# ml-unito/PartitionedLS.jl

Measured on NVIDIA B200. Metric: opt_fit_orthant_nnls_solves_per_sec, higher is better.
Workload: dtype f64

## Files before the change

partitionedls.jl_b200/csrc/nnls5.cu:

```cuda
#include "common.cuh"

namespace pls {
namespace {

constexpr int H5_BYTES_ = 192;
constexpr int SG_FREE5 = 2;
constexpr unsigned char ST_INO = 1;
constexpr unsigned char ST_PAS = 2;
constexpr unsigned char ST_BLK = 4;
constexpr unsigned char ST_FAST = 8;
#define SYNC5() __syncthreads()

__device__ __forceinline__ void dmma5(double &d0, double &d1, double a, double b) {
  asm("mma.sync.aligned.m8n8k4.row.col.f64.f64.f64.f64 {%0,%1}, {%2}, {%3}, {%0,%1};\n"
      : "+d"(d0), "+d"(d1) : "d"(a), "d"(b));
}
__device__ __forceinline__ double rcp5(double x) {
  double r;
  asm("rcp.approx.ftz.f64 %0, %1;" : "=d"(r) : "d"(x));
  double e = fma(-x, r, 1.0);
  r = fma(r, e, r);
  e = fma(-x, r, 1.0);
  return fma(r, e, r);
}
__device__ __forceinline__ double wsum5(double v) {
#pragma unroll
  for (int o = 16; o; o >>= 1) v += __shfl_xor_sync(0xffffffffu, v, o);
  return v;
}
__device__ __forceinline__ double wmax5(double v) {
#pragma unroll
  for (int o = 16; o; o >>= 1) v = fmax(v, __shfl_xor_sync(0xffffffffu, v, o));
  return v;
}
__host__ __device__ constexpr int t2_doubles(int nr) { return ((nr / 8) * (nr / 8 + 1) / 2) * 64; }
__device__ __forceinline__ int t2_idx(int i, int j) {
  const int ti = i >> 3, tj = j >> 3;
  return ((((ti * (ti + 1)) >> 1) + tj) << 6) + ((i & 7) << 3) + (j & 7);
}
__device__ __forceinline__ double t2_get(const double *T2, int i, int j) { return i >= j ? T2[t2_idx(i, j)] : T2[t2_idx(j, i)]; }
__device__ __forceinline__ void t2_set(double *T2, int i, int j, double v) {
  const int a = i > j ? i : j, b = i > j ? j : i;
  const int x = t2_idx(a, b);
  T2[x] = v;
  if ((a >> 3) == (b >> 3)) T2[x - ((a & 7) << 3) - (b & 7) + ((b & 7) << 3) + (a & 7)] = v;
}
__device__ __forceinline__ int pan5(int row, int col) { return (row << 3) + (col ^ ((row & 2) << 1)); }

struct Sh5 {
  double *T2;
  double *v;
  double *Pp, *Wp;
  double *yv;
  double *D;
  double *gd;
  double *red;
  int4 *binfo;
  int *ctl;
  short *slot;
  short *rvar;
  short *lst;
  short *lstE;
  short *lstB;
  unsigned short *tmap;
  signed char *sg;
  unsigned char *st;
  unsigned char *grp;
  unsigned char *mk;
};
enum { C_NS = 0, C_OK, C_CNT, C_N, C_NJ, C_NP, C_NLV, C_FLAG };

__host__ __device__ inline size_t sh5_bytes(int NR, int ld1) {
  const int ntl = (NR / 8) * (NR / 8 + 1) / 2;
  return H5_BYTES_ + sizeof(double) * ((size_t)t2_doubles(NR) + ld1 + 16 * (size_t)NR + NR + 64 + 8 + 32 + 16) + sizeof(int) * 16 +
         sizeof(short) * (2 * (size_t)ld1 + 2 * (size_t)NR + 8 + ((ntl + 3) & ~3)) + 3 * (size_t)ld1 + NR + 16 + 16;
}

__device__ __forceinline__ Sh5 make_sh5(int NR, int ld1) {
  extern __shared__ __align__(16) unsigned char smem_raw5[];
  const int ntl = (NR / 8) * (NR / 8 + 1) / 2;
  Sh5 s;
  double *dp = reinterpret_cast<double *>(smem_raw5 + H5_BYTES_);
  s.T2 = dp; dp += t2_doubles(NR);
  s.Pp = dp; dp += 8 * NR;
  s.Wp = dp; dp += 8 * NR;
  s.yv = dp; dp += NR;
  s.D = dp; dp += 64;
  s.gd = dp; dp += 8;
  s.red = dp; dp += 32;
  s.binfo = reinterpret_cast<int4 *>(dp); dp += 16;
  int *ip = reinterpret_cast<int *>(dp);
  s.ctl = ip; ip += 16;
  short *sp = reinterpret_cast<short *>(ip);
  s.rvar = sp; sp += NR;
  s.lstE = sp; sp += NR;
  s.lstB = sp; sp += 8;
  s.tmap = reinterpret_cast<unsigned short *>(sp); sp += (ntl + 3) & ~3;
  s.mk = reinterpret_cast<unsigned char *>(sp);
  dp = reinterpret_cast<double *>(smem_raw5 + ((static_cast<int>(s.mk - smem_raw5) + NR + 15) & ~15));
  s.v = dp; dp += ld1;
  sp = reinterpret_cast<short *>(dp);
  s.slot = sp; sp += ld1;
  s.lst = sp; sp += ld1;
  signed char *cp = reinterpret_cast<signed char *>(sp);
  s.sg = cp; cp += ld1;
  s.st = reinterpret_cast<unsigned char *>(cp); cp += ld1;
  s.grp = reinterpret_cast<unsigned char *>(cp);
  return s;
}

struct H5 {
  double *T1;
  const double *T1r;
  double *Pg;
  const double *G;
  const unsigned long long *gmask;
  int ld1, nr, Mp, ldg;
  int cold_fused;
  int gen;
  int pad0, pad1;
  unsigned long long cnt[10];
  double yy, cmax;
  double max_viol;
};
enum { H_SWEEP = 0, H_STREAM, H_SUMS, H_SUMP2, H_ITER, H_BLK, H_REBUILD, H_FOLD, H_DRIFT, H_NOCONV };
constexpr int H5_BYTES = H5_BYTES_;
static_assert(sizeof(H5) <= H5_BYTES, "header size");
__device__ __forceinline__ H5 &hdr5() {
  extern __shared__ __align__(16) unsigned char smem_raw5[];
  return *reinterpret_cast<H5 *>(smem_raw5);
}

template <int T>
__device__ __forceinline__ double bmax5(const Sh5 &s, double v) {
  constexpr int NW = T / 32;
  v = wmax5(v);
  if ((threadIdx.x & 31) == 0) s.red[threadIdx.x >> 5] = v;
  SYNC5();
  double r = s.red[0];
#pragma unroll
  for (int i = 1; i < NW; ++i) r = fmax(r, s.red[i]);
  SYNC5();
  return r;
}

template <int T>
__device__ __forceinline__ void set_block5(const Sh5 &s, int nb, int slot) {
  const int tid = threadIdx.x;
  const H5 &h = hdr5();
  const int g = h.gen;
  if (g == 1) {
    #pragma unroll 1
    for (int k = tid; k < h.nr; k += T) s.mk[k] = 0;
    SYNC5();
  }
  if (tid < nb) {
    const int tc = slot >> 3, c7 = slot & 7;
    s.lstB[tid] = (short)slot;
    s.binfo[tid] = make_int4(slot, (tc << 6) + c7, (((tc * (tc + 1)) >> 1) << 6) + (c7 << 3), 0);
    s.mk[slot] = (unsigned char)g;
  }
}

template <int T, int NR>
__device__ __noinline__ int t2_block(int n, int nb, int nlv, bool test, bool flip) {
  H5 &h = hdr5();
  const int gen = h.gen;
  const Sh5 s = make_sh5(NR, h.ld1);
  constexpr int NW = T / 32;
  const int tid = threadIdx.x, lane = tid & 31, wid = tid >> 5;
  const int fr = lane >> 2, fk = lane & 3;
  const int ntr = (n + 7) >> 3;
  const short *B = s.lstB;
  if (tid >= 32 || T == 32) {
    constexpr int TG = T == 32 ? 32 : T - 32;
#pragma unroll 1
    for (int row = T == 32 ? tid : tid - 32; row < ntr * 8; row += TG) {
      const int tr = row >> 3, r7 = row & 7;
      const int rbase = (((tr * (tr + 1)) >> 1) << 6) + (r7 << 3), rowt = (tr << 6) + r7;
      const int sw = (row & 2) << 1, pb = row << 3;
#pragma unroll 1
      for (int q = 0; q < 8; ++q) {
        double val = 0.0;
        if (row < n && q < nb) { const int4 bi = s.binfo[q]; val = s.T2[row >= bi.x ? rbase + bi.y : bi.z + rowt]; }
        s.Pp[pb + (q ^ sw)] = val;
      }
    }
  }
  if (tid < 32) {
    if (lane < 8) {
      s.gd[lane] = (test && lane >= nlv && lane < nb) ? 1e-13 * __ldg(h.G + (size_t)h.ldg * s.rvar[B[lane]] + s.rvar[B[lane]]) : 0.0;
    }
    const int i = lane >> 2, j0 = (lane & 3) << 1;
    double e0 = (i < nb && j0 < nb) ? t2_get(s.T2, B[i], B[j0]) : (i == j0 ? 1.0 : 0.0);
    double e1 = (i < nb && j0 + 1 < nb) ? t2_get(s.T2, B[i], B[j0 + 1]) : (i == j0 + 1 ? 1.0 : 0.0);
    int bad = nb;
#pragma unroll 1
    for (int k = 0; k < nb; ++k) {
      __syncwarp();
      s.D[i * 8 + j0] = e0; s.D[i * 8 + j0 + 1] = e1;
      __syncwarp();
      const double pk0 = s.D[k * 8 + j0], pk1 = s.D[k * 8 + j0 + 1], cik = s.D[i * 8 + k], pkk = s.D[k * 8 + k];
      const bool good = k < nlv ? pkk < 0.0 : (test ? pkk > s.gd[k] : pkk > 0.0);
      if (!good && bad == nb) bad = k;
      const double d = rcp5(pkk), fct = cik * d;
      const bool rowk = i == k;
      double n0 = rowk ? pk0 * d : fma(-fct, pk0, e0);
      double n1 = rowk ? pk1 * d : fma(-fct, pk1, e1);
      if (j0 == k) n0 = rowk ? d : -fct;
      if (j0 + 1 == k) n1 = rowk ? d : -fct;
      e0 = n0; e1 = n1;
    }
    __syncwarp();
    s.D[i * 8 + j0] = e0; s.D[i * 8 + j0 + 1] = e1;
    if (lane == 0) s.ctl[C_OK] = bad == nb ? nb : (bad < nlv ? -1 : bad);
  }
  SYNC5();
  const int res = s.ctl[C_OK];
  if (tid == 0) h.gen = gen == 255 ? 1 : gen + 1;
  if (res != nb) { SYNC5(); return res; }
  #pragma unroll 1
  for (int ti = wid; ti < ntr; ti += NW) {
    double c0 = 0.0, c1 = 0.0;
    dmma5(c0, c1, s.Pp[pan5(ti * 8 + fr, fk)], s.D[fk * 8 + fr]);
    dmma5(c0, c1, s.Pp[pan5(ti * 8 + fr, 4 + fk)], s.D[(4 + fk) * 8 + fr]);
    *reinterpret_cast<double2 *>(s.Wp + pan5(ti * 8 + fr, 2 * fk)) = make_double2(c0, c1);
  }
  SYNC5();
  {
    const int ntl = (ntr * (ntr + 1)) >> 1;
    int q = (ntl * wid) / NW;
    const int q1 = (ntl * (wid + 1)) / NW;
    const int t0 = s.tmap[q];
    int ti = t0 >> 8, tj = t0 & 255;
    const int la0 = pan5(fr, fk), la1 = pan5(fr, 4 + fk);
    double2 *cp = reinterpret_cast<double2 *>(s.T2 + (q << 6) + fr * 8 + 2 * fk);
    const double *pw = s.Wp + (ti << 6), *pp = s.Pp + (tj << 6);
    double a0 = -pw[la0], a1 = -pw[la1];
#pragma unroll 1
    for (; q < q1; ++q) {
      double2 c0 = *cp;
      dmma5(c0.x, c0.y, a0, pp[la0]);
      dmma5(c0.x, c0.y, a1, pp[la1]);
      *cp = c0;
      cp += 32; pp += 64;
      if (++tj > ti) { ++ti; tj = 0; pp = s.Pp; pw += 64; a0 = -pw[la0]; a1 = -pw[la1]; }
    }
  }
  SYNC5();
#pragma unroll 1
  for (int row = tid; row < n; row += T) {
    if (s.mk[row] == (unsigned char)gen) continue;
    const int tr = row >> 3, r7 = row & 7;
    const int rbase = (((tr * (tr + 1)) >> 1) << 6) + (r7 << 3), rowt = (tr << 6) + r7;
    const int sw = (row & 2) << 1, pb = row << 3;
#pragma unroll 1
    for (int q = 0; q < nb; ++q) {
      const int4 bi = s.binfo[q];
      const int tc = bi.x >> 3;
      const double w0 = s.Wp[pb + (q ^ sw)];
      const double val = q < nlv ? -w0 : w0;
      if (tr >= tc) s.T2[rbase + bi.y] = val;
      if (tr <= tc) s.T2[bi.z + rowt] = val;
    }
  }
#pragma unroll 1
  for (int e = tid; e < 64; e += T) {
    const int i = e >> 3, j = e & 7;
    if (i < nb && j <= i) { const double val = s.D[i * 8 + j]; t2_set(s.T2, B[i], B[j], ((i < nlv) == (j < nlv)) ? -val : val); }
  }
  if (flip && tid < nb) s.st[s.rvar[B[tid]]] ^= ST_PAS;
  SYNC5();
  if (tid == 0) { h.cnt[H_SWEEP] += nb; h.cnt[H_SUMP2] += ((unsigned long long)(n * n) * nb) >> 2; }
  return nb;
}

template <int T, int NR>
__device__ __noinline__ bool t2_rebuild(int n) {
  const H5 &h = hdr5();
  const Sh5 s = make_sh5(NR, h.ld1);
  constexpr int NW = T / 32;
  const int tid = threadIdx.x, lane = tid & 31, wid = tid >> 5;
  #pragma unroll 1
  for (int i = wid; i < n; i += NW) {
    const double *row = h.T1r + (size_t)h.ld1 * s.rvar[i];
    #pragma unroll 1
    for (int j = lane; j <= i; j += 32) t2_set(s.T2, i, j, __ldcg(row + s.rvar[j]));
  }
  if (tid < 32) {
    int cnt = 0, nlv = 0;
    #pragma unroll 1
    for (int pass = 0; pass < 2; ++pass) {
      #pragma unroll 1
      for (int k0 = 1; k0 < n; k0 += 32) {
        const int k = k0 + lane;
        bool take = false;
        if (k < n) { const unsigned char f = s.st[s.rvar[k]]; const bool pas = f & ST_PAS, ino = f & ST_INO; take = pas != ino && (pass == 0 ? !pas : pas); }
        const unsigned bal = __ballot_sync(0xffffffffu, take);
        if (take) s.lst[cnt + __popc(bal & ((1u << lane) - 1))] = (short)k;
        cnt += __popc(bal);
      }
      if (pass == 0) nlv = cnt;
    }
    if (lane == 0) { s.ctl[C_CNT] = cnt; s.ctl[C_NLV] = nlv; }
  }
  SYNC5();
  const int cnt = s.ctl[C_CNT], nlv = s.ctl[C_NLV];
  #pragma unroll 1
  for (int q0 = 0; q0 < cnt; q0 += 8) {
    const int nb = min(8, cnt - q0);
    set_block5<T>(s, nb, tid < nb ? s.lst[q0 + tid] : 0);
    SYNC5();
    if (t2_block<T, NR>(n, nb, max(0, min(nb, nlv - q0)), false, false) != nb) return false;
  }
  return true;
}

template <int NR>
__device__ __noinline__ int window_reset() {
  const H5 &h = hdr5();
  const Sh5 s = make_sh5(NR, h.ld1);
  const int tid = threadIdx.x;
  const int Mp = h.Mp;
  if (tid < 32) {
    const int lane = tid;
    if (lane == 0) s.rvar[0] = (short)Mp;
    int base = 1;
    #pragma unroll 1
    for (int m0 = 0; m0 < Mp; m0 += 32) {
      const int m = m0 + lane;
      bool keep = false;
      if (m < Mp) {
        const unsigned char f = s.st[m];
        keep = (f & ST_FAST) || (((f & ST_PAS) != 0) != ((f & ST_INO) != 0));
      }
      const unsigned bal = __ballot_sync(0xffffffffu, keep);
      if (m < Mp) {
        if (keep) { const int k = base + __popc(bal & ((1u << lane) - 1)); s.rvar[k] = (short)m; s.slot[m] = (short)k; }
        else s.slot[m] = -1;
      }
      base += __popc(bal);
    }
    if (lane == 0) s.ctl[C_N] = base;
  }
  SYNC5();
  return s.ctl[C_N];
}

template <int T, int NR>
__device__ __noinline__ int t2_compact(int n) {
  const H5 &h = hdr5();
  const Sh5 s = make_sh5(NR, h.ld1);
  const int tid = threadIdx.x;
  double *scr = h.Pg + 8 * (size_t)h.ld1;
  short *old = s.lst;
  if (tid < 32) {
    const int lane = tid;
    if (lane == 0) old[0] = 0;
    int base = 1;
    #pragma unroll 1
    for (int k0 = 1; k0 < n; k0 += 32) {
      const int k = k0 + lane;
      bool keep = false; int m = 0;
      if (k < n) {
        m = s.rvar[k];
        const unsigned char f = s.st[m];
        keep = (f & ST_FAST) || (((f & ST_PAS) != 0) != ((f & ST_INO) != 0));
      }
      const unsigned bal = __ballot_sync(0xffffffffu, keep);
      const int kn = base + __popc(bal & ((1u << lane) - 1));
      __syncwarp();
      if (k < n) {
        if (keep) { old[kn] = (short)k; s.rvar[kn] = (short)m; s.slot[m] = (short)kn; }
        else s.slot[m] = -1;
      }
      __syncwarp();
      base += __popc(bal);
    }
    if (lane == 0) s.ctl[C_N] = base;
  }
  SYNC5();
  const int nn = s.ctl[C_N];
  if (nn == n) return n;
  #pragma unroll 1
  for (int idx = tid; idx < nn * nn; idx += T) {
    const int a = idx / nn, b = idx - a * nn;
    if (b <= a) __stcg(scr + idx, t2_get(s.T2, old[a], old[b]));
  }
  __threadfence_block();
  SYNC5();
  #pragma unroll 1
  for (int idx = tid; idx < nn * nn; idx += T) {
    const int a = idx / nn, b = idx - a * nn;
    if (b <= a) t2_set(s.T2, a, b, __ldcg(scr + idx));
  }
  SYNC5();
  return nn;
}

template <int T, int NQ, int NR>
__device__ __noinline__ void stream5(int n) {
  const H5 &h = hdr5();
  const Sh5 s = make_sh5(NR, h.ld1);
  const int tid = threadIdx.x;
  const int ld2 = h.ld1 >> 1;
  constexpr int UB = 8;
  constexpr int NG = T >= 512 ? 2 : 1, TG = T / NG, NQE = NQ * NG, UBG = UB * NG;
  const int grp = NG == 1 ? 0 : tid / TG, lt = NG == 1 ? tid : tid - grp * TG;
  int ns = 0;
  {
    constexpr int NW = T / 32;
    const int lane = tid & 31, wid = tid >> 5;
    int *ri = reinterpret_cast<int *>(s.red);
    #pragma unroll 1
    for (int k0 = 1; k0 < n; k0 += T) {
      const int k = k0 + tid;
      bool tg = false, pas = false; int m = 0;
      if (k < n) { m = s.rvar[k]; const unsigned char f = s.st[m]; pas = f & ST_PAS; tg = pas != ((f & ST_INO) != 0); }
      const unsigned bal = __ballot_sync(0xffffffffu, tg);
      if (k0 > 1) SYNC5();
      if (lane == 0) ri[wid] = __popc(bal);
      SYNC5();
      int off = ns;
#pragma unroll
      for (int w2 = 0; w2 < NW; ++w2) { const int c = ri[w2]; if (w2 < wid) off += c; ns += c; }
      if (tg) { const int p = off + __popc(bal & ((1u << lane) - 1)); s.lst[p] = (short)m; const double t = s.T2[t2_idx(k, 0)]; s.yv[p] = pas ? t : -t; }
    }
    const int nsp = (ns + UBG - 1) / UBG * UBG;
    #pragma unroll 1
    for (int p = ns + tid; p < nsp; p += T) { s.lst[p] = (short)h.Mp; s.yv[p] = 0.0; }
    if (tid == 0) { s.ctl[C_NS] = ns; s.ctl[C_FLAG] = 0; }
  }
  SYNC5();
  const int nsp = (ns + UBG - 1) / UBG * UBG;
  double2 acc[NQE];
  const double2 *T1v = reinterpret_cast<const double2 *>(h.T1r);
  {
    const double2 *r = T1v + (size_t)ld2 * h.Mp;
#pragma unroll
    for (int q = 0; q < NQE; ++q) acc[q] = (grp == 0 && lt + TG * q < ld2) ? __ldcg(r + lt + TG * q) : make_double2(0.0, 0.0);
  }
  #pragma unroll 1
  for (int p = 0; p < nsp; p += UBG) {
    double2 g[UB][NQE];
#pragma unroll
    for (int u = 0; u < UB; ++u) {
      const double2 *r = T1v + (size_t)ld2 * s.lst[p + u * NG + grp];
#pragma unroll
      for (int q = 0; q < NQE; ++q) g[u][q] = (lt + TG * q < ld2) ? __ldcg(r + lt + TG * q) : make_double2(0.0, 0.0);
    }
#pragma unroll
    for (int u = 0; u < UB; ++u) {
      const double y = s.yv[p + u * NG + grp];
#pragma unroll
      for (int q = 0; q < NQE; ++q) { acc[q].x = fma(-y, g[u][q].x, acc[q].x); acc[q].y = fma(-y, g[u][q].y, acc[q].y); }
    }
  }
  if (NG > 1) {
    double2 *scr = reinterpret_cast<double2 *>(s.Wp);
    if (grp == 1) {
#pragma unroll
      for (int q = 0; q < NQE; ++q) if (lt + TG * q < ld2) scr[lt + TG * q] = acc[q];
    }
    SYNC5();
    if (grp == 0) {
#pragma unroll
      for (int q = 0; q < NQE; ++q) if (lt + TG * q < ld2) { const double2 o = scr[lt + TG * q]; acc[q].x += o.x; acc[q].y += o.y; }
    }
  }
  if (grp == 0) {
#pragma unroll
    for (int q = 0; q < NQE; ++q)
      if (lt + TG * q < ld2) reinterpret_cast<double2 *>(s.v)[lt + TG * q] = acc[q];
  }
  SYNC5();
  if (tid == 0) { hdr5().cnt[H_STREAM]++; hdr5().cnt[H_SUMS] += ns; }
}

template <int T, int NR>
__device__ __noinline__ void join5(int n, int m) {
  const H5 &h = hdr5();
  const Sh5 s = make_sh5(NR, h.ld1);
  const int tid = threadIdx.x;
  const double *row1 = h.T1r + (size_t)h.ld1 * m;
  double *rowv = s.Wp, *tog = s.Wp + NR;
  int ns = 0;
  {
    constexpr int NW = T / 32;
    const int lane = tid & 31, wid = tid >> 5;
    int *ri = reinterpret_cast<int *>(s.red);
    #pragma unroll 1
    for (int k0 = 1; k0 < n; k0 += T) {
      const int k = k0 + tid;
      bool tg = false, pas = false; int var = 0;
      if (k < n) { var = s.rvar[k]; const unsigned char f = s.st[var]; pas = f & ST_PAS; tg = pas != ((f & ST_INO) != 0); }
      const unsigned bal = __ballot_sync(0xffffffffu, tg);
      if (k0 > 1) SYNC5();
      if (lane == 0) ri[wid] = __popc(bal);
      SYNC5();
      int off = ns;
#pragma unroll
      for (int w2 = 0; w2 < NW; ++w2) { const int c = ri[w2]; if (w2 < wid) off += c; ns += c; }
      if (tg) { const int p = off + __popc(bal & ((1u << lane) - 1)); s.lstE[p] = (short)k; const double a = __ldcg(row1 + var); s.yv[p] = pas ? a : -a; }
      if (k < n) tog[k] = tg ? 1.0 : 0.0;
    }
    if (tid == 0) tog[0] = 0.0;
  }
  SYNC5();
  #pragma unroll 1
  for (int j = tid; j < n; j += T) {
    double a = tog[j] != 0.0 ? 0.0 : __ldcg(row1 + s.rvar[j]);
    #pragma unroll 1
    for (int p = 0; p < ns; ++p) a = fma(-s.yv[p], t2_get(s.T2, s.lstE[p], j), a);
    rowv[j] = a;
  }
  SYNC5();
  #pragma unroll 1
  for (int j = tid; j < n; j += T) t2_set(s.T2, n, j, rowv[j]);
  if (tid < 32) {
    double dg = 0.0;
    #pragma unroll 1
    for (int p = tid; p < ns; p += 32) dg = fma(s.yv[p], rowv[s.lstE[p]], dg);
    dg = wsum5(dg);
    if (tid == 0) { t2_set(s.T2, n, n, __ldcg(row1 + m) - dg); s.rvar[n] = (short)m; s.slot[m] = (short)n; }
  }
  if (tid == 0) hdr5().cnt[H_SUMP2] += (unsigned long long)(ns * n) >> 1;
  SYNC5();
}

template <int T, int NR>
__device__ __noinline__ bool fold_block5(int boff, int nb) {
  H5 &h = hdr5();
  const Sh5 s = make_sh5(NR, h.ld1);
  const short *B = s.lstE + boff;
  constexpr int NW = T / 32;
  const int tid = threadIdx.x, lane = tid & 31, wid = tid >> 5;
  const int fr = lane >> 2, fk = lane & 3;
  const int ld1 = h.ld1, nt = ld1 >> 3;
  double *FP = s.T2, *FW = s.T2 + (size_t)ld1 * 8;
  #pragma unroll 1
  for (int idx = tid; idx < ld1 * 8; idx += T) {
    const int j = idx >> 3, q = idx & 7;
    FP[pan5(j, q)] = q < nb ? __ldcg(h.T1r + (size_t)ld1 * B[q] + j) : 0.0;
  }
  if (tid < 8) s.gd[tid] = (tid < nb && (s.st[B[tid]] & ST_PAS)) ? 1e-13 * __ldg(h.G + (size_t)h.ldg * B[tid] + B[tid]) : 0.0;
  SYNC5();
  if (tid < 32) {
    bool ok = true;
    const int i = lane >> 2, j0 = (lane & 3) << 1;
    double e0 = (i < nb && j0 < nb) ? FP[pan5(B[i], j0)] : (i == j0 ? 1.0 : 0.0);
    double e1 = (i < nb && j0 + 1 < nb) ? FP[pan5(B[i], j0 + 1)] : (i == j0 + 1 ? 1.0 : 0.0);
    #pragma unroll 1
    for (int k = 0; k < nb; ++k) {
      __syncwarp();
      s.D[i * 8 + j0] = e0; s.D[i * 8 + j0 + 1] = e1;
      __syncwarp();
      const double pk0 = s.D[k * 8 + j0], pk1 = s.D[k * 8 + j0 + 1], cik = s.D[i * 8 + k], pkk = s.D[k * 8 + k];
      if (s.st[B[k]] & ST_PAS) ok = ok && pkk > s.gd[k];
      else ok = ok && pkk < 0.0;
      const double d = 1.0 / pkk, fct = cik * d;
      const bool rowk = i == k;
      double n0 = rowk ? pk0 * d : fma(-fct, pk0, e0);
      double n1 = rowk ? pk1 * d : fma(-fct, pk1, e1);
      if (j0 == k) n0 = rowk ? d : -fct;
      if (j0 + 1 == k) n1 = rowk ? d : -fct;
      e0 = n0; e1 = n1;
    }
    __syncwarp();
    s.D[i * 8 + j0] = e0; s.D[i * 8 + j0 + 1] = e1;
    ok = __all_sync(0xffffffffu, ok);
    if (lane == 0) s.ctl[C_OK] = ok ? 1 : 0;
  }
  SYNC5();
  if (!s.ctl[C_OK]) { SYNC5(); return false; }
  #pragma unroll 1
  for (int ti = wid; ti < nt; ti += NW) {
    double c0 = 0.0, c1 = 0.0;
    dmma5(c0, c1, FP[pan5(ti * 8 + fr, fk)], s.D[fk * 8 + fr]);
    dmma5(c0, c1, FP[pan5(ti * 8 + fr, 4 + fk)], s.D[(4 + fk) * 8 + fr]);
    *reinterpret_cast<double2 *>(FW + pan5(ti * 8 + fr, 2 * fk)) = make_double2(c0, c1);
  }
  SYNC5();
  {
    const int ntl = (nt * (nt + 1)) >> 1;
    constexpr int IFL = (T <= 64 || T >= 512) ? 8 : 4;
    int q = (ntl * wid) / NW;
    const int q1 = (ntl * (wid + 1)) / NW;
    int ti = 0;
    while (((ti + 1) * (ti + 2)) >> 1 <= q) ++ti;
    int tj = q - ((ti * (ti + 1)) >> 1);
    #pragma unroll 1
    for (; q < q1; q += IFL) {
      double2 c[IFL]; int ri[IFL], rj[IFL];
#pragma unroll
      for (int u = 0; u < IFL; ++u) {
        ri[u] = ti; rj[u] = tj;
        c[u] = __ldcg(reinterpret_cast<const double2 *>(h.T1r + (size_t)(ti * 8 + fr) * ld1 + tj * 8 + 2 * fk));
        if (q + u + 1 < q1) { if (++tj > ti) { ++ti; tj = 0; } }
      }
#pragma unroll
      for (int u = 0; u < IFL; ++u) {
        const int ra = ri[u] * 8 + fr, rb = rj[u] * 8 + fr;
        dmma5(c[u].x, c[u].y, -FW[pan5(ra, fk)], FP[pan5(rb, fk)]);
        dmma5(c[u].x, c[u].y, -FW[pan5(ra, 4 + fk)], FP[pan5(rb, 4 + fk)]);
      }
#pragma unroll
      for (int u = 0; u < IFL; ++u) {
        if (q + u < q1) {
          __stcg(reinterpret_cast<double2 *>(h.T1 + (size_t)(ri[u] * 8 + fr) * ld1 + rj[u] * 8 + 2 * fk), c[u]);
          if (ri[u] != rj[u]) {
            double *mp = h.T1 + (size_t)(rj[u] * 8 + 2 * fk) * ld1 + ri[u] * 8 + fr;
            __stcg(mp, c[u].x); __stcg(mp + ld1, c[u].y);
          }
        }
      }
    }
  }
  SYNC5();
  #pragma unroll 1
  for (int idx = tid; idx < ld1 * 8; idx += T) {
    const int i = idx >> 3, q = idx & 7;
    if (q < nb) {
      const double val = (s.st[B[q]] & ST_PAS) ? FW[pan5(i, q)] : -FW[pan5(i, q)];
      __stcg(h.T1 + (size_t)ld1 * B[q] + i, val);
      __stcg(h.T1 + (size_t)ld1 * i + B[q], val);
    }
  }
  SYNC5();
  #pragma unroll 1
  for (int e = tid; e < 64; e += T) {
    const int i = e >> 3, j = e & 7;
    if (i < nb && j < nb) {
      const double ei = (s.st[B[i]] & ST_PAS) ? 1.0 : -1.0, ej = (s.st[B[j]] & ST_PAS) ? 1.0 : -1.0;
      __stcg(h.T1 + (size_t)ld1 * B[i] + B[j], -ei * ej * s.D[i * 8 + j]);
    }
  }
  SYNC5();
  if (tid < nb) { const int m = B[tid]; const unsigned char f = s.st[m]; s.st[m] = (f & ST_PAS) ? (unsigned char)(f | ST_INO) : (unsigned char)(f & ~ST_INO); }
  if (tid == 0) { h.T1r = h.T1; h.cnt[H_SUMP2] += 2ull * ld1 * ld1; h.cnt[H_FOLD]++; }
  SYNC5();
  return true;
}

template <int T, int NR>
__device__ __noinline__ void fold_fused5(int n) {
  H5 &h = hdr5();
  const Sh5 s = make_sh5(NR, h.ld1);
  constexpr int NW = T / 32;
  const int tid = threadIdx.x, lane = tid & 31, wid = tid >> 5;
  const int fr = lane >> 2, fk = lane & 3;
  const int ld1 = h.ld1, nt = ld1 >> 3;
  const int ntr = (n + 7) >> 3, nk = ntr << 3;
  double *PR = h.Pg + 8 * (size_t)ld1, *ZT = PR + (size_t)ld1 * h.nr;
  int *roff = reinterpret_cast<int *>(s.Wp);
  const bool own = h.T1r == h.T1;
  const double *rows = own ? PR : h.T1r;
  #pragma unroll 1
  for (int k = tid; k < nk; k += T) {
    double e = 0.0;
    if (k >= 1 && k < n) { const unsigned char f = s.st[s.rvar[k]]; const bool pas = f & ST_PAS, ino = f & ST_INO; if (pas != ino) e = pas ? 1.0 : -1.0; }
    s.yv[k] = e;
    roff[k] = e != 0.0 ? (own ? k : (int)s.rvar[k]) * ld1 : 0;
  }
  SYNC5();
  if (own) {
    #pragma unroll 1
    for (int k = 0; k < n; ++k) {
      if (k > 0 && s.yv[k] == 0.0) continue;
      const double *src = h.T1 + (size_t)ld1 * (s.yv[k] != 0.0 ? s.rvar[k] : 0);
      #pragma unroll 1
      for (int j = tid; j < ld1; j += T) PR[(size_t)k * ld1 + j] = __ldcg(src + j);
    }
    __threadfence_block();
    SYNC5();
  }
  constexpr int NTQ = 12;
#pragma unroll 1
  for (int tj = wid; tj < nt; tj += NW) {
    const double *pa = rows + tj * 8 + fr;
    double2 acc[NTQ];
#pragma unroll
    for (int u = 0; u < NTQ; ++u) acc[u] = make_double2(0.0, 0.0);
    double a0 = s.yv[fk] * __ldcg(pa + roff[fk]), a1 = s.yv[4 + fk] * __ldcg(pa + roff[4 + fk]);
#pragma unroll 1
    for (int tk = 0; tk < ntr; ++tk) {
      double n0 = 0.0, n1 = 0.0;
      if (tk + 1 < ntr) { const int k = (tk + 1) * 8 + fk; n0 = s.yv[k] * __ldcg(pa + roff[k]); n1 = s.yv[k + 4] * __ldcg(pa + roff[k + 4]); }
#pragma unroll
      for (int tq = 0; tq < NTQ; ++tq) {
        if (tq < ntr) {
          double b0, b1;
          if (tk >= tq) { const double *tp = s.T2 + ((((tk * (tk + 1)) >> 1) + tq) << 6); b0 = tp[fk * 8 + fr]; b1 = tp[(4 + fk) * 8 + fr]; }
          else { const double *tp = s.T2 + ((((tq * (tq + 1)) >> 1) + tk) << 6); b0 = tp[fr * 8 + fk]; b1 = tp[fr * 8 + 4 + fk]; }
          dmma5(acc[tq].x, acc[tq].y, a0, b0); dmma5(acc[tq].x, acc[tq].y, a1, b1);
        }
      }
      a0 = n0; a1 = n1;
    }
#pragma unroll
    for (int tq = 0; tq < NTQ; ++tq)
      if (tq < ntr) {
        const int k = tq * 8 + 2 * fk;
        *reinterpret_cast<double2 *>(ZT + (size_t)(tj * 8 + fr) * nk + k) = make_double2(acc[tq].x * s.yv[k], acc[tq].y * s.yv[k + 1]);
      }
  }
  __threadfence_block();
  SYNC5();
  constexpr int CH = 5;
  {
    const int ntl = (nt * (nt + 1)) >> 1;
    int q = (ntl * wid) / NW;
    const int q1 = (ntl * (wid + 1)) / NW;
    int ti = 0;
    while (((ti + 1) * (ti + 2)) >> 1 <= q) ++ti;
    int tj = q - ((ti * (ti + 1)) >> 1);
    #pragma unroll 1
    for (; q < q1; ++q) {
      double2 c = __ldcg(reinterpret_cast<const double2 *>(h.T1r + (size_t)(ti * 8 + fr) * ld1 + tj * 8 + 2 * fk));
      const double *za = ZT + (size_t)(ti * 8 + fr) * nk + fk, *pb = rows + tj * 8 + fr;
#pragma unroll 1
      for (int t0 = 0; t0 < ntr; t0 += CH) {
        double z0[CH], z1[CH], p0[CH], p1[CH];
#pragma unroll
        for (int u = 0; u < CH; ++u) {
          const bool live = t0 + u < ntr;
          const int k = (t0 + u) * 8 + fk;
          z0[u] = live ? za[(t0 + u) * 8] : 0.0; z1[u] = live ? za[(t0 + u) * 8 + 4] : 0.0;
          p0[u] = live ? __ldcg(pb + roff[k]) : 0.0; p1[u] = live ? __ldcg(pb + roff[k + 4]) : 0.0;
        }
#pragma unroll
        for (int u = 0; u < CH; ++u) { dmma5(c.x, c.y, z0[u], p0[u]); dmma5(c.x, c.y, z1[u], p1[u]); }
      }
      __stcg(reinterpret_cast<double2 *>(h.T1 + (size_t)(ti * 8 + fr) * ld1 + tj * 8 + 2 * fk), c);
      if (ti != tj) {
        double *mp = h.T1 + (size_t)(tj * 8 + 2 * fk) * ld1 + ti * 8 + fr;
        __stcg(mp, c.x); __stcg(mp + ld1, c.y);
      }
      if (++tj > ti) { ++ti; tj = 0; }
    }
  }
  SYNC5();
  #pragma unroll 1
  for (int k = 1; k < n; ++k) {
    const double e = s.yv[k];
    if (e == 0.0) continue;
    const int var = s.rvar[k];
    #pragma unroll 1
    for (int j = tid; j < ld1; j += T) {
      const double val = -e * ZT[(size_t)j * nk + k];
      __stcg(h.T1 + (size_t)ld1 * var + j, val);
      __stcg(h.T1 + (size_t)ld1 * j + var, val);
    }
  }
  SYNC5();
  #pragma unroll 1
  for (int idx = tid; idx < n * n; idx += T) {
    const int a = idx / n, b = idx - a * n;
    __stcg(h.T1 + (size_t)ld1 * s.rvar[a] + s.rvar[b], t2_get(s.T2, a, b));
  }
  SYNC5();
  #pragma unroll 1
  for (int k = tid; k < n; k += T) {
    if (k >= 1 && s.yv[k] != 0.0) { const int m = s.rvar[k]; const unsigned char f = s.st[m]; s.st[m] = (f & ST_PAS) ? (unsigned char)(f | ST_INO) : (unsigned char)(f & ~ST_INO); }
  }
  if (tid == 0) { h.T1r = h.T1; h.cnt[H_SUMP2] += 2ull * ld1 * ld1 * (unsigned long long)ntr / 8 + (unsigned long long)ld1 * nk * nk / 2; h.cnt[H_FOLD]++; }
  SYNC5();
}

template <int T, int NR>
__device__ __noinline__ int fold5(int n, bool cold_mode) {
  const H5 &h = hdr5();
  const Sh5 s = make_sh5(NR, h.ld1);
  const int tid = threadIdx.x;
  if (cold_mode) n = t2_compact<T, NR>(n);
  short *B = s.lstE;
  if (tid < 32) {
    const int lane = tid;
    int cnt = 0;
    #pragma unroll 1
    for (int pass = 0; pass < 2; ++pass) {
      #pragma unroll 1
      for (int k0 = 1; k0 < n; k0 += 32) {
        const int k = k0 + lane;
        bool take = false; int m = 0;
        if (k < n) {
          m = s.rvar[k];
          const unsigned char f = s.st[m];
          const bool pas = f & ST_PAS, ino = f & ST_INO;
          take = pas != ino && !(f & ST_FAST) && (pass == 0 ? !pas : pas);
        }
        const unsigned bal = __ballot_sync(0xffffffffu, take);
        if (take) B[cnt + __popc(bal & ((1u << lane) - 1))] = (short)m;
        cnt += __popc(bal);
      }
    }
    if (lane == 0) s.ctl[C_CNT] = cnt;
  }
  SYNC5();
  const int cnt = s.ctl[C_CNT];
  bool ok = true;
  if (cold_mode && cnt > 8 && h.cold_fused) fold_fused5<T, NR>(n);
  else for (int q0 = 0; q0 < cnt && ok; q0 += 8) ok = fold_block5<T, NR>(q0, min(8, cnt - q0));
  n = window_reset<NR>();
  if (!t2_rebuild<T, NR>(n)) ok = false;
  return ok ? n : -1;
}

// ... 41 lines not shown
    else if (sg == SG_FREE5) mx = fmax(mx, fabs(rv));
    else if (sg != 0 && !(f & ST_BLK)) mx = fmax(mx, (double)sg * rv);
  }
  return bmax5<T>(s, mx);
}

template <int T, int NR, int NQ>
__device__ __forceinline__ bool solve5(const Sh5 s, int &n_win, bool cold_mode, bool &t2_fresh) {
  const int tid = threadIdx.x;
  H5 &h = hdr5();
  const int Mp = h.Mp;
  const double cmax = h.cmax;
  const double told = 1e-12 * cmax;
  int t_best = Mp + 1, pbar = 3, iters = 0, rebuilt = 0;
  #pragma unroll 1
  for (;;) {
    #pragma unroll 1
    for (;;) {
      const int n = n_win;
      int nl = 0, ne = 0, mx = -1;
      {
        constexpr int NW = T / 32;
        const int lane = tid & 31, wid = tid >> 5;
        int4 *ri = reinterpret_cast<int4 *>(s.red);
        #pragma unroll 1
        for (int k0 = 1; k0 < n; k0 += T) {
          const int k = k0 + tid;
          int f = 0, m = -1;
          if (k < n) {
            m = s.rvar[k];
            const double val = s.T2[t2_idx(k, 0)];
            const int sg = s.sg[m];
            const unsigned char fl = s.st[m];
            if (fl & ST_PAS) { if (sg != SG_FREE5 && (sg == 0 || (double)sg * val < 0.0)) f = 1; }
            else if (!(fl & ST_BLK) && sg != 0 && (sg == SG_FREE5 ? fabs(val) > told : (double)sg * val > told)) f = 2;
          }
          const unsigned bl = __ballot_sync(0xffffffffu, f == 1), be = __ballot_sync(0xffffffffu, f == 2);
          const int mw = __reduce_max_sync(0xffffffffu, f ? m : -1);
          if (k0 > 1) SYNC5();
          if (lane == 0) ri[wid] = make_int4(__popc(bl), __popc(be), mw, 0);
          SYNC5();
          int ol = nl, oe = ne;
#pragma unroll
          for (int w2 = 0; w2 < NW; ++w2) {
            const int4 r = ri[w2];
            if (w2 < wid) { ol += r.x; oe += r.y; }
            nl += r.x; ne += r.y; mx = max(mx, r.z);
          }
          const unsigned below = (1u << lane) - 1;
          if (f == 1) s.lst[ol + __popc(bl & below)] = (short)k;
          if (f == 2) s.lstE[oe + __popc(be & below)] = (short)k;
        }
      }
      SYNC5();
      const int nv = nl + ne;
      if (nv == 0) break;
      if (tid == 0) h.cnt[H_ITER]++;
      if (++iters > 60 + 6 * Mp) return false;
      bool single = false;
      if (nv < t_best) { t_best = nv; pbar = 3; }
      else if (pbar >= 1) --pbar;
      else single = true;
      if (single) {
        const int k = s.slot[mx];
        const bool pas = s.st[mx] & ST_PAS;
        nl = pas ? 1 : 0; ne = pas ? 0 : 1;
        SYNC5();
        if (tid == 0) { if (pas) s.lst[0] = (short)k; else s.lstE[0] = (short)k; }
        SYNC5();
      }
      t2_fresh = false;
      int done = 0, tot = nl + ne;
      bool broken = false;
      while (done < tot) {
        const int nb = min(8, tot - done), nlv = max(0, min(nb, nl - done));
        set_block5<T>(s, nb, tid < nb ? (done + tid < nl ? s.lst[done + tid] : s.lstE[done + tid - nl]) : 0);
        SYNC5();
        const int r = t2_block<T, NR>(n, nb, nlv, true, true);
        if (r == nb) { done += nb; continue; }
        if (r < 0) { broken = true; break; }
        const int pos = done + r - nl;
        if (tid == 0) {
          s.st[s.rvar[s.lstE[pos]]] |= ST_BLK;
          #pragma unroll 1
          for (int q = pos; q + 1 < ne; ++q) s.lstE[q] = s.lstE[q + 1];
        }
        --ne; --tot; if (tid == 0) h.cnt[H_BLK]++;
        SYNC5();
      }
      if (broken) {
        if (++rebuilt > 3 || !t2_rebuild<T, NR>(n)) return false;
        t2_fresh = true; if (tid == 0) h.cnt[H_REBUILD]++;
      }
    }
    stream5<T, NQ, NR>(n_win);
    {
      const int ns = s.ctl[C_NS];
      int code = 0;
#pragma unroll 1
      for (int p = tid; p < ns; p += T) if (!(fabs(s.v[s.lst[p]]) <= 1e-12 * cmax)) code |= 2;
#pragma unroll 1
      for (int m = tid; m < Mp; m += T) {
        if (s.slot[m] < 0) {
          const int sg = s.sg[m];
          const unsigned char fl = s.st[m];
          const double val = s.v[m];
          bool f;
          if (fl & ST_INO) f = sg != SG_FREE5 && (sg == 0 ? val != 0.0 : (double)sg * val < 0.0);
          else f = !(fl & ST_BLK) && sg != 0 && (sg == SG_FREE5 ? fabs(val) > told : (double)sg * val > told);
          if (f) code |= 1;
        }
      }
      if (code) atomicOr(&s.ctl[C_FLAG], code);
      SYNC5();
      const int flags = s.ctl[C_FLAG];
      if (flags & 2) {
        double res = 0.0;
#pragma unroll 1
        for (int p = tid; p < ns; p += T) { const double r = fabs(s.v[s.lst[p]]); res = r == r ? fmax(res, r) : r; }
        res = bmax5<T>(s, res);
        if (res != res || (t2_fresh && res > 1e-9 * cmax) || ++rebuilt > 3) return false;
        if (!t2_rebuild<T, NR>(n_win)) return false;
        t2_fresh = true;
        if (tid == 0) h.cnt[H_REBUILD]++;
        continue;
      }
      if (!(flags & 1)) return true;
    }
    if (tid < 32) {
      const int lane = tid;
      int nj = 0;
#pragma unroll 1
      for (int m0 = 0; m0 < Mp; m0 += 32) {
        const int m = m0 + lane;
        bool f = false;
        if (m < Mp && s.slot[m] < 0) {
          const int sg = s.sg[m];
          const unsigned char fl = s.st[m];
          const double val = s.v[m];
          if (fl & ST_INO) f = sg != SG_FREE5 && (sg == 0 ? val != 0.0 : (double)sg * val < 0.0);
          else f = !(fl & ST_BLK) && sg != 0 && (sg == SG_FREE5 ? fabs(val) > told : (double)sg * val > told);
        }
        const unsigned bal = __ballot_sync(0xffffffffu, f);
        if (f) s.lst[nj + __popc(bal & ((1u << lane) - 1))] = (short)m;
        nj += __popc(bal);
      }
      if (lane == 0) s.ctl[C_NJ] = nj;
    }
    SYNC5();
    const int nj = s.ctl[C_NJ];
    if (nj == 0) return true;
    if (++iters > 60 + 6 * Mp) return false;
    if (NR - n_win < nj) {
      short *park = reinterpret_cast<short *>(s.v);
      #pragma unroll 1
      for (int p = tid; p < nj; p += T) park[p] = s.lst[p];
      SYNC5();
      if (cold_mode) n_win = t2_compact<T, NR>(n_win);
      if (NR - n_win < (nj < 8 ? nj : 8)) {
        const int nf = fold5<T, NR>(n_win, cold_mode);
        if (nf < 0) return false;
        n_win = nf;
        t2_fresh = true;
      }
      int room = NR - n_win;
      if (room > nj) room = nj;
      if (room <= 0) return false;
      #pragma unroll 1
      for (int p = 0; p < room; ++p) { const int m = park[p]; if (s.slot[m] < 0) { join5<T, NR>(n_win, m); ++n_win; } }
    } else {
      #pragma unroll 1
      for (int p = 0; p < nj; ++p) { join5<T, NR>(n_win, s.lst[p]); ++n_win; }
    }
    t_best = Mp + 1; pbar = 3;
  }
}

template <int T, int NR>
__device__ __noinline__ void cold_init5(const double *T0) {
  H5 &h = hdr5();
  const Sh5 s = make_sh5(NR, h.ld1);
  const int tid = threadIdx.x, ld1 = h.ld1;
  if (tid == 0) h.T1r = T0;
  #pragma unroll 1
  for (int m = tid; m < ld1; m += T) { s.st[m] = 0; s.slot[m] = -1; s.sg[m] = 0; }
  SYNC5();
}

__global__ void __launch_bounds__(128) k2v5_build_t0(const double *G, int ldg, const double *c, const double *scal, int Mp, int ld1, double *T0) {
  const int row = blockIdx.x;
  for (int col = threadIdx.x; col < ld1; col += blockDim.x) {
    double val = 0.0;
    if (row < Mp) val = col < Mp ? G[(size_t)ldg * row + col] : (col == Mp ? c[row] : 0.0);
    else if (row == Mp) val = col < Mp ? c[col] : (col == Mp ? scal[0] : 0.0);
    T0[(size_t)ld1 * row + col] = val;
  }
}

template <int T>
__device__ __forceinline__ void set_lowmask5(const Sh5 &s, unsigned long long mask) {
  const H5 &h = hdr5();
  #pragma unroll 1
  for (int m = threadIdx.x; m < h.Mp; m += T) {
    const unsigned char f = s.st[m];
    s.st[m] = (h.gmask[m] & mask) ? (unsigned char)(f | ST_FAST) : (unsigned char)(f & ~ST_FAST);
  }
  SYNC5();
}

template <int T>
__device__ __forceinline__ void set_signs5(const Sh5 &s, long long b, int free_top, int Kp, int fb) {
  const H5 &h = hdr5();
  #pragma unroll 1
  for (int m = threadIdx.x; m < h.Mp; m += T) {
    const int g = s.grp[m];
    if (fb >= 0 && g != 255) {
      if (g == fb) s.sg[m] = (signed char)-s.sg[m];
    } else if (fb < 0 || ((h.gmask[m] >> fb) & 1ull)) {
      const unsigned long long gm = h.gmask[m];
      const int d = 2 * __popcll(gm & (unsigned long long)b) - __popcll(gm);
      const bool fr = free_top && ((gm >> (Kp - 1)) & 1ull);
      s.sg[m] = (signed char)(fr ? SG_FREE5 : (d > 0) - (d < 0));
    }
    s.st[m] &= (unsigned char)~ST_BLK;
  }
  SYNC5();
}

template <int T, int NR, int NQ, int MINB>
__global__ void __launch_bounds__(T, MINB) k2v5_orthant_walks(const K2Args A) {
  const int tid = threadIdx.x;
  const int Mp = A.Mp, ld1 = A.cap;
  const Sh5 s = make_sh5(NR, ld1);
  H5 &h = hdr5();
  if (tid == 0) {
    h.T1 = A.tab + (size_t)blockIdx.x * A.tabstride; h.ld1 = ld1; h.T1r = A.hglob;
    h.Pg = h.T1 + (size_t)ld1 * ld1;
    h.Mp = Mp; h.nr = NR; h.cold_fused = A.chain_log2; h.gen = 1;
    h.gmask = reinterpret_cast<const unsigned long long *>(A.gmask);
    h.G = A.G; h.ldg = A.ldg;
    #pragma unroll 1
    for (int q = 0; q < 10; ++q) h.cnt[q] = 0;
    h.yy = A.scal[0]; h.cmax = A.scal[1]; h.max_viol = 0.0;
  }
  int n_win = 1;
  bool cold_mode = true;
  #pragma unroll 1
  for (int ti = tid; ti < NR / 8; ti += T)
    #pragma unroll 1
    for (int tj = 0; tj <= ti; ++tj) s.tmap[((ti * (ti + 1)) >> 1) + tj] = (unsigned short)((ti << 8) | tj);
  #pragma unroll 1
  for (int k = tid; k < NR; k += T) s.mk[k] = 0;
  #pragma unroll 1
  for (int m = tid; m < Mp; m += T) { const unsigned long long gm = reinterpret_cast<const unsigned long long *>(A.gmask)[m]; s.grp[m] = (unsigned char)(__popcll(gm) == 1 ? __ffsll((long long)gm) - 1 : 255); }
  #pragma unroll 1
  for (int e = tid; e < t2_doubles(NR); e += T) s.T2[e] = 0.0;
  double best_obj = 0.0; long long best_b = -1;
  int low_bits = 0;
  while ((A.lowmask >> low_bits) & 1ull) ++low_bits;
  const long long cnt = A.n_chains;
  const long long i0 = cnt * (long long)blockIdx.x / (long long)gridDim.x;
  const long long i1 = cnt * ((long long)blockIdx.x + 1) / (long long)gridDim.x;
  bool cold = true, just_cold = false, t2_fresh = true;
  int since_check = 0, check_every = A.verify_every;
  SYNC5();

  #pragma unroll 1
  for (long long i = i0; i < i1; ++i) {
    if (cold) {
      cold_init5<T, NR>(A.hglob);
      cold_mode = true;
      n_win = window_reset<NR>();
      t2_rebuild<T, NR>(n_win);
      cold = false; just_cold = true; since_check = 0; t2_fresh = true;
    }
    const long long b = A.b_begin + (i ^ (i >> 1));
    const int fb = i > 0 ? __ffsll(i) - 1 : 63;
    set_signs5<T>(s, b, A.free_top, A.Kp, (just_cold || i == i0) ? -1 : fb);

    const bool ok = solve5<T, NR, NQ>(s, n_win, cold_mode, t2_fresh);
    if (!ok) { cold = true; if (tid == 0) h.cnt[H_NOCONV]++; }

    ++since_check;
    if (ok && (since_check >= check_every || i + 1 == i1)) {
      since_check = 0;
      const double viol = verify5<T, NR>(A.c);
      const double cmax = h.cmax;
      if (!just_cold && tid == 0) h.max_viol = fmax(h.max_viol, viol);
      if (viol > 1e-13 * cmax && check_every > 8) check_every = 8;
      if (viol > 1e-12 * cmax && !just_cold) { if (tid == 0) h.cnt[H_DRIFT]++; cold = true; --i; continue; }
    }
    just_cold = false;

    const double obj = ok ? sqrt(fmax(s.v[Mp], 0.0)) : __longlong_as_double(0x7ff8000000000000ll);
    const long long rel = b - A.b_begin;
    double w_top = 0.0;
    if (A.free_top && (s.st[Mp - 1] & ST_PAS)) w_top = s.slot[Mp - 1] >= 0 ? s.T2[t2_idx(s.slot[Mp - 1], 0)] : s.v[Mp - 1];
    const long long b_full = A.free_top ? (b | ((w_top > 0.0 ? 1ll : 0ll) << (A.Kp - 1))) : b;
    if (A.all_obj && tid == 0) A.all_obj[rel] = obj;
    const bool better = opt_better(obj, b_full, best_obj, best_b, PLS_TIE_REL * h.yy);
    if (better) { best_obj = obj; best_b = b_full; }
    if (A.all_alpha || better) {
      #pragma unroll 1
      for (int m = tid; m < Mp; m += T) {
        const unsigned long long gm = h.gmask[m];
        const int d = 2 * __popcll(gm & (unsigned long long)b) - __popcll(gm);
        double wv = 0.0;
        if (ok && (s.st[m] & ST_PAS)) wv = s.slot[m] >= 0 ? s.T2[t2_idx(s.slot[m], 0)] : s.v[m];
        const double al = s.sg[m] == SG_FREE5 ? fabs(wv) : (d != 0 ? fmax(wv / (double)d, 0.0) : 0.0);
        if (A.all_alpha) A.all_alpha[(size_t)rel * Mp + m] = al;
        if (better) A.cta_w[(size_t)blockIdx.x * Mp + m] = al;
      }
    }
    if (ok) {
      bool tslow = false;
#pragma unroll 1
      for (int k = tid + 1; k < n_win; k += T) {
        const int m = s.rvar[k]; const unsigned char f = s.st[m];
        tslow = tslow || ((((f & ST_PAS) != 0) != ((f & ST_INO) != 0)) && !(f & ST_FAST));
      }
      const int nslow = __syncthreads_count(tslow);
      const bool was_cold = cold_mode;
      if (fb >= low_bits || nslow >= 8 || n_win > NR - 8 || was_cold) {
        const int nf = fold5<T, NR>(n_win, cold_mode);
        if (nf < 0) cold = true;
        else n_win = nf;
        t2_fresh = true;
        if (was_cold && !cold) {
          set_lowmask5<T>(s, A.lowmask);
          cold_mode = false;
          n_win = window_reset<NR>();
          if (!t2_rebuild<T, NR>(n_win)) cold = true;
        }
      }
    }
    SYNC5();
  }
  if (tid == 0) {
    A.cta_obj[blockIdx.x] = best_obj;
    A.cta_b[blockIdx.x] = best_b;
    atomicAdd(&A.counters[CNT_PIVOTS], h.cnt[H_SWEEP]);
    atomicAdd(&A.counters[CNT_GRAD], h.cnt[H_STREAM]);
    atomicAdd(&A.counters[CNT_SUMP], h.cnt[H_SUMS]);
    atomicAdd(&A.counters[CNT_SUMP2], h.cnt[H_SUMP2]);
    atomicAdd(&A.counters[CNT_ITERS], h.cnt[H_ITER]);
    atomicAdd(&A.counters[CNT_REBUILDS], h.cnt[H_REBUILD]);
    atomicAdd(&A.counters[CNT_BLOCKED], h.cnt[H_BLK]);
    atomicAdd(&A.counters[CNT_NOCONV], h.cnt[H_NOCONV]);
    atomicAdd(&A.counters[CNT_SPILLS], h.cnt[H_DRIFT]);
    atomicMax(&A.counters[CNT_DRIFT], (unsigned long long)__double_as_longlong(h.max_viol / h.cmax));
    atomicAdd(&A.counters[CNT_V5_FOLDS], h.cnt[H_FOLD]);
  }
}

typedef void (*K5Fn)(const K2Args);
struct Variant5 { int T, NR, NQ, minb; K5Fn fn; };
#define V5(T, NR, NQ, MINB) {T, NR, NQ, MINB, k2v5_orthant_walks<T, NR, NQ, MINB>}
const Variant5 kVariants5[] = {
    V5(128, 64, 1, 7), V5(128, 72, 1, 6), V5(128, 80, 1, 5), V5(128, 96, 1, 4), V5(64, 64, 2, 7), V5(64, 72, 2, 6), V5(64, 80, 2, 5), V5(64, 96, 2, 4),
    V5(32, 72, 4, 6),
    V5(128, 96, 2, 4),
    V5(512, 160, 1, 1), V5(512, 192, 1, 1), V5(512, 208, 1, 1),
};
#undef V5

}

int k2v5_plan(int Mp, int n_bits, const uint64_t *h_gmask, K5Plan *pl) {
  if (!h_gmask) return PLS_EUNSUPPORTED;
  const int ld1 = (Mp + 1 + 7) & ~7;
  const char *eT = getenv("PLS_K5_T"), *eN = getenv("PLS_K5_NR");
  const int wantT = eT ? atoi(eT) : 0, wantNR = eN ? atoi(eN) : 0;
  int dev = 0, max_smem = 0;
  PLS_CUDA_TRY(cudaGetDevice(&dev));
  PLS_CUDA_TRY(cudaDeviceGetAttribute(&max_smem, cudaDevAttrMaxSharedMemoryPerBlockOptin, dev));
  const Variant5 *v = nullptr;
  int vi = -1, l = 0;
  const char *eM = getenv("PLS_K5_MARGIN");
  const int margin = eM ? atoi(eM) : 12;
  const int l_want = n_bits - 2 < 6 ? (n_bits - 2 < 1 ? 1 : n_bits - 2) : 6;
  int ci = 0;
  for (const Variant5 &c : kVariants5) {
    const bool fits = c.T == (wantT ? wantT : (ld1 > 328 ? 512 : 128)) && (!wantNR || c.NR == wantNR) && ld1 <= 2 * c.T * c.NQ &&
                      2 * (size_t)ld1 * 8 <= (size_t)t2_doubles(c.NR) + 16 * (size_t)c.NR && sh5_bytes(c.NR, ld1) <= (size_t)max_smem;
    if (fits) {
      int lc = 0;
      for (int t = 1; t <= n_bits && t <= 10; ++t) {
        int nf = 0;
        const uint64_t mask = (1ull << t) - 1ull;
        for (int m = 0; m < Mp; ++m) nf += (h_gmask[m] & mask) != 0ull;
        if (nf + 1 + margin <= c.NR) lc = t; else break;
      }
      if (lc > l) { v = &c; vi = ci; l = lc; }
      if (l >= l_want) break;
    }
    ++ci;
  }
  if (!v || l < 1) return PLS_EUNSUPPORTED;
  if (const char *eL = getenv("PLS_K5_L")) { const int t = atoi(eL); if (t >= 1 && t < l) l = t; }
  const size_t sm = sh5_bytes(v->NR, ld1);
  PLS_CUDA_TRY(cudaFuncSetAttribute(v->fn, cudaFuncAttributeMaxDynamicSharedMemorySize, (int)sm));
  int oc = 1;
  PLS_CUDA_TRY(cudaOccupancyMaxActiveBlocksPerMultiprocessor(&oc, v->fn, v->T, sm));
  if (oc < 1) oc = 1;
  if (const char *eO = getenv("PLS_K5_OCC")) { const int o = atoi(eO); if (o >= 1 && o < oc) oc = o; }
  pl->variant = vi; pl->T = v->T; pl->NR = v->NR; pl->ld1 = ld1; pl->occ = oc; pl->smem = sm; pl->low_groups = l;
  pl->tabstride = (size_t)ld1 * ld1 + 8 * (size_t)ld1 + 2 * (size_t)ld1 * v->NR + 64;
  const char *eV = getenv("PLS_K5_VERIFY");
  pl->verify_every = eV ? atoi(eV) : 128;
  const char *eF = getenv("PLS_K5_FUSED");
  pl->cold_fused = v->NR > 96 ? 0 : (eF ? atoi(eF) : 1);
  if (pl->verify_every < 1) pl->verify_every = 1;
  return PLS_OK;
}

int k2v5_launch(const K2Args &A, const K5Plan &pl, int grid, cudaStream_t st) {
  k2v5_build_t0<<<pl.ld1, 128, 0, st>>>(A.G, A.ldg, A.c, A.scal, A.Mp, pl.ld1, A.hglob);
  PLS_CUDA_TRY(cudaGetLastError());
  kVariants5[pl.variant].fn<<<grid, pl.T, pl.smem, st>>>(A);
  PLS_CUDA_TRY(cudaGetLastError());
  return PLS_OK;
}

}
```

Measured before the change: 35.43 million.

## Eliminate Wp and v shared buffers by aliasing onto Pp to shrink smem

Removes the separate Wp (8*NR doubles) and v (ld1 doubles) shared-memory buffers. v now aliases Pp, and the W=P*D panel product is computed on the fly inside the trailing update, then written back over Pp afterwards. The row-join path drops its temporary rowv/tog arrays by recomputing the toggle from state flags and writing straight into T2. Parked join indices move to global scratch. The smaller footprint is meant to allow more blocks per SM or larger NR variants, at the cost of recomputing W per tile row, extra syncs and global traffic when parking.

```diff
diff --git a/partitionedls.jl_b200/csrc/nnls5.cu b/partitionedls.jl_b200/csrc/nnls5.cu
--- a/partitionedls.jl_b200/csrc/nnls5.cu
+++ b/partitionedls.jl_b200/csrc/nnls5.cu
@@ -49,8 +49,8 @@
 
 struct Sh5 {
   double *T2;
+  double *Pp;
   double *v;
-  double *Pp, *Wp;
   double *yv;
   double *D;
   double *gd;
@@ -72,8 +72,8 @@
 
 __host__ __device__ inline size_t sh5_bytes(int NR, int ld1) {
   const int ntl = (NR / 8) * (NR / 8 + 1) / 2;
-  return H5_BYTES_ + sizeof(double) * ((size_t)t2_doubles(NR) + ld1 + 16 * (size_t)NR + NR + 64 + 8 + 32 + 16) + sizeof(int) * 16 +
-         sizeof(short) * (2 * (size_t)ld1 + 2 * (size_t)NR + 8 + ((ntl + 3) & ~3)) + 3 * (size_t)ld1 + NR + 16 + 16;
+  return H5_BYTES_ + sizeof(double) * ((size_t)t2_doubles(NR) + 8 * (size_t)NR + NR + 64 + 8 + 32 + 16) + sizeof(int) * 16 +
+         sizeof(short) * (2 * (size_t)ld1 + 2 * (size_t)NR + 8 + ((ntl + 3) & ~3)) + 3 * (size_t)ld1 + NR + 16;
 }
 
 __device__ __forceinline__ Sh5 make_sh5(int NR, int ld1) {
@@ -83,7 +83,7 @@
   double *dp = reinterpret_cast<double *>(smem_raw5 + H5_BYTES_);
   s.T2 = dp; dp += t2_doubles(NR);
   s.Pp = dp; dp += 8 * NR;
-  s.Wp = dp; dp += 8 * NR;
+  s.v = s.Pp;
   s.yv = dp; dp += NR;
   s.D = dp; dp += 64;
   s.gd = dp; dp += 8;
@@ -96,10 +96,7 @@
   s.lstE = sp; sp += NR;
   s.lstB = sp; sp += 8;
   s.tmap = reinterpret_cast<unsigned short *>(sp); sp += (ntl + 3) & ~3;
-  s.mk = reinterpret_cast<unsigned char *>(sp);
-  dp = reinterpret_cast<double *>(smem_raw5 + ((static_cast<int>(s.mk - smem_raw5) + NR + 15) & ~15));
-  s.v = dp; dp += ld1;
-  sp = reinterpret_cast<short *>(dp);
+  s.mk = reinterpret_cast<unsigned char *>(sp); sp += NR / 2;
   s.slot = sp; sp += ld1;
   s.lst = sp; sp += ld1;
   signed char *cp = reinterpret_cast<signed char *>(sp);
@@ -219,15 +216,9 @@
   const int res = s.ctl[C_OK];
   if (tid == 0) h.gen = gen == 255 ? 1 : gen + 1;
   if (res != nb) { SYNC5(); return res; }
-  #pragma unroll 1
-  for (int ti = wid; ti < ntr; ti += NW) {
-    double c0 = 0.0, c1 = 0.0;
-    dmma5(c0, c1, s.Pp[pan5(ti * 8 + fr, fk)], s.D[fk * 8 + fr]);
-    dmma5(c0, c1, s.Pp[pan5(ti * 8 + fr, 4 + fk)], s.D[(4 + fk) * 8 + fr]);
-    *reinterpret_cast<double2 *>(s.Wp + pan5(ti * 8 + fr, 2 * fk)) = make_double2(c0, c1);
-  }
-  SYNC5();
   {
+    const int pc = (fr >> 1) + ((fr & 1) << 2);
+    const double d0 = s.D[fk * 8 + pc], d1 = s.D[(4 + fk) * 8 + pc];
     const int ntl = (ntr * (ntr + 1)) >> 1;
     int q = (ntl * wid) / NW;
     const int q1 = (ntl * (wid + 1)) / NW;
@@ -235,8 +226,10 @@
     int ti = t0 >> 8, tj = t0 & 255;
     const int la0 = pan5(fr, fk), la1 = pan5(fr, 4 + fk);
     double2 *cp = reinterpret_cast<double2 *>(s.T2 + (q << 6) + fr * 8 + 2 * fk);
-    const double *pw = s.Wp + (ti << 6), *pp = s.Pp + (tj << 6);
-    double a0 = -pw[la0], a1 = -pw[la1];
+    const double *pw = s.Pp + (ti << 6), *pp = s.Pp + (tj << 6);
+    double a0 = 0.0, a1 = 0.0;
+    dmma5(a0, a1, pw[la0], d0); dmma5(a0, a1, pw[la1], d1);
+    a0 = -a0; a1 = -a1;
 #pragma unroll 1
     for (; q < q1; ++q) {
       double2 c0 = *cp;
@@ -244,8 +237,22 @@
       dmma5(c0.x, c0.y, a1, pp[la1]);
       *cp = c0;
       cp += 32; pp += 64;
-      if (++tj > ti) { ++ti; tj = 0; pp = s.Pp; pw += 64; a0 = -pw[la0]; a1 = -pw[la1]; }
-    }
+      if (++tj > ti && q + 1 < q1) {
+        ++ti; tj = 0; pp = s.Pp; pw += 64;
+        a0 = 0.0; a1 = 0.0;
+        dmma5(a0, a1, pw[la0], d0); dmma5(a0, a1, pw[la1], d1);
+        a0 = -a0; a1 = -a1;
+      }
+    }
+  }
+  SYNC5();
+  #pragma unroll 1
+  for (int ti = wid; ti < ntr; ti += NW) {
+    double c0 = 0.0, c1 = 0.0;
+    dmma5(c0, c1, s.Pp[pan5(ti * 8 + fr, fk)], s.D[fk * 8 + fr]);
+    dmma5(c0, c1, s.Pp[pan5(ti * 8 + fr, 4 + fk)], s.D[(4 + fk) * 8 + fr]);
+    __syncwarp();
+    *reinterpret_cast<double2 *>(s.Pp + pan5(ti * 8 + fr, 2 * fk)) = make_double2(c0, c1);
   }
   SYNC5();
 #pragma unroll 1
@@ -258,7 +265,7 @@
     for (int q = 0; q < nb; ++q) {
       const int4 bi = s.binfo[q];
       const int tc = bi.x >> 3;
-      const double w0 = s.Wp[pb + (q ^ sw)];
+      const double w0 = s.Pp[pb + (q ^ sw)];
       const double val = q < nlv ? -w0 : w0;
       if (tr >= tc) s.T2[rbase + bi.y] = val;
       if (tr <= tc) s.T2[bi.z + rowt] = val;
@@ -457,7 +464,7 @@
     }
   }
   if (NG > 1) {
-    double2 *scr = reinterpret_cast<double2 *>(s.Wp);
+    double2 *scr = reinterpret_cast<double2 *>(s.v);
     if (grp == 1) {
 #pragma unroll
       for (int q = 0; q < NQE; ++q) if (lt + TG * q < ld2) scr[lt + TG * q] = acc[q];
@@ -483,7 +490,6 @@
   const Sh5 s = make_sh5(NR, h.ld1);
   const int tid = threadIdx.x;
   const double *row1 = h.T1r + (size_t)h.ld1 * m;
-  double *rowv = s.Wp, *tog = s.Wp + NR;
   int ns = 0;
   {
     constexpr int NW = T / 32;
@@ -502,25 +508,24 @@
 #pragma unroll
       for (int w2 = 0; w2 < NW; ++w2) { const int c = ri[w2]; if (w2 < wid) off += c; ns += c; }
       if (tg) { const int p = off + __popc(bal & ((1u << lane) - 1)); s.lstE[p] = (short)k; const double a = __ldcg(row1 + var); s.yv[p] = pas ? a : -a; }
-      if (k < n) tog[k] = tg ? 1.0 : 0.0;
-    }
-    if (tid == 0) tog[0] = 0.0;
+    }
   }
   SYNC5();
   #pragma unroll 1
   for (int j = tid; j < n; j += T) {
-    double a = tog[j] != 0.0 ? 0.0 : __ldcg(row1 + s.rvar[j]);
+    const int var = s.rvar[j];
+    const unsigned char f = s.st[var];
+    const bool tg = j > 0 && ((f & ST_PAS) != 0) != ((f & ST_INO) != 0);
+    double a = tg ? 0.0 : __ldcg(row1 + var);
     #pragma unroll 1
     for (int p = 0; p < ns; ++p) a = fma(-s.yv[p], t2_get(s.T2, s.lstE[p], j), a);
-    rowv[j] = a;
-  }
-  SYNC5();
-  #pragma unroll 1
-  for (int j = tid; j < n; j += T) t2_set(s.T2, n, j, rowv[j]);
+    t2_set(s.T2, n, j, a);
+  }
+  SYNC5();
   if (tid < 32) {
     double dg = 0.0;
     #pragma unroll 1
-    for (int p = tid; p < ns; p += 32) dg = fma(s.yv[p], rowv[s.lstE[p]], dg);
+    for (int p = tid; p < ns; p += 32) dg = fma(s.yv[p], s.T2[t2_idx(n, s.lstE[p])], dg);
     dg = wsum5(dg);
     if (tid == 0) { t2_set(s.T2, n, n, __ldcg(row1 + m) - dg); s.rvar[n] = (short)m; s.slot[m] = (short)n; }
   }
@@ -652,7 +657,7 @@
   const int ld1 = h.ld1, nt = ld1 >> 3;
   const int ntr = (n + 7) >> 3, nk = ntr << 3;
   double *PR = h.Pg + 8 * (size_t)ld1, *ZT = PR + (size_t)ld1 * h.nr;
-  int *roff = reinterpret_cast<int *>(s.Wp);
+  int *roff = reinterpret_cast<int *>(s.Pp);
   const bool own = h.T1r == h.T1;
   const double *rows = own ? PR : h.T1r;
   #pragma unroll 1
@@ -1000,9 +1005,10 @@
     if (nj == 0) return true;
     if (++iters > 60 + 6 * Mp) return false;
     if (NR - n_win < nj) {
-      short *park = reinterpret_cast<short *>(s.v);
+      int *park = reinterpret_cast<int *>(h.Pg);
       #pragma unroll 1
-      for (int p = tid; p < nj; p += T) park[p] = s.lst[p];
+      for (int p = tid; p < nj; p += T) __stcg(park + p, (int)s.lst[p]);
+      __threadfence_block();
       SYNC5();
       if (cold_mode) n_win = t2_compact<T, NR>(n_win);
       if (NR - n_win < (nj < 8 ? nj : 8)) {
@@ -1015,7 +1021,10 @@
       if (room > nj) room = nj;
       if (room <= 0) return false;
       #pragma unroll 1
-      for (int p = 0; p < room; ++p) { const int m = park[p]; if (s.slot[m] < 0) { join5<T, NR>(n_win, m); ++n_win; } }
+      for (int p = tid; p < room; p += T) s.lst[p] = (short)__ldcg(park + p);
+      SYNC5();
+      #pragma unroll 1
+      for (int p = 0; p < room; ++p) { const int m = s.lst[p]; if (s.slot[m] < 0) { join5<T, NR>(n_win, m); ++n_win; } }
     } else {
       #pragma unroll 1
       for (int p = 0; p < nj; ++p) { join5<T, NR>(n_win, s.lst[p]); ++n_win; }
@@ -1230,7 +1239,8 @@
   int ci = 0;
   for (const Variant5 &c : kVariants5) {
     const bool fits = c.T == (wantT ? wantT : (ld1 > 328 ? 512 : 128)) && (!wantNR || c.NR == wantNR) && ld1 <= 2 * c.T * c.NQ &&
-                      2 * (size_t)ld1 * 8 <= (size_t)t2_doubles(c.NR) + 16 * (size_t)c.NR && sh5_bytes(c.NR, ld1) <= (size_t)max_smem;
+                      2 * (size_t)ld1 * 8 <= (size_t)t2_doubles(c.NR) + 8 * (size_t)c.NR && ld1 <= 8 * c.NR &&
+                      sh5_bytes(c.NR, ld1) <= (size_t)max_smem;
     if (fits) {
       int lc = 0;
       for (int t = 1; t <= n_bits && t <= 10; ++t) {
```

Result: no change. 35.34 million (median of 6 runs) (-0.3%).
